# majidsina/rlmd

Hardware: NVIDIA B200
Metric: investor-steps/sec (leverage sweep) (higher is better)
Workload: dtype 2-bit codes, int32 counts, f64 log-wealth, f32 wealth

## Files before the change

rlmd_b200/csrc/common.cuh:

```cuda
#pragma once

#include <cuda_runtime.h>
#include <stdint.h>

#include <cstdarg>
#include <cstdio>

#include "../../include/rlmd_b200.h"

namespace b200 {

int set_error(int code, const char* fmt, ...);
int check_cuda(cudaError_t e, const char* what);

#define B200_CUDA(expr)                                   \
  do {                                                    \
    int _rc = ::b200::check_cuda((expr), #expr);          \
    if (_rc != 0) return _rc;                             \
  } while (0)

#define B200_REQUIRE(cond, ...)                                     \
  do {                                                              \
    if (!(cond)) return ::b200::set_error(B200_EINVAL, __VA_ARGS__); \
  } while (0)

int sm_count();

struct Philox4 {
  uint32_t x, y, z, w;
};

__host__ __device__ __forceinline__ uint32_t mulhi32(uint32_t a, uint32_t b) {
#ifdef __CUDA_ARCH__
  return __umulhi(a, b);
#else
  return (uint32_t)(((uint64_t)a * (uint64_t)b) >> 32);
#endif
}

__host__ __device__ __forceinline__ Philox4 philox4x32_10(uint32_t c0, uint32_t c1, uint32_t c2,
                                                           uint32_t c3, uint32_t k0, uint32_t k1) {
  const uint32_t M0 = 0xD2511F53u, M1 = 0xCD9E8D57u;
  const uint32_t W0 = 0x9E3779B9u, W1 = 0xBB67AE85u;
#pragma unroll
  for (int r = 0; r < 10; ++r) {
    uint32_t hi0 = mulhi32(M0, c0), lo0 = M0 * c0;
    uint32_t hi1 = mulhi32(M1, c2), lo1 = M1 * c2;
    uint32_t n0 = hi1 ^ c1 ^ k0;
    uint32_t n2 = hi0 ^ c3 ^ k1;
    c0 = n0;
    c1 = lo1;
    c2 = n2;
    c3 = lo0;
    k0 += W0;
    k1 += W1;
  }
  return Philox4{c0, c1, c2, c3};
}

// ... 150 lines not shown
```

rlmd_b200/csrc/lev_sweep.cu:

```cuda
#include <cstdlib>

#include "lev_kernels.cuh"
#include "tally.cuh"

namespace b200 {

struct LogFactorTable {
  double lm[B200_MAX_OUTCOMES][B200_MAX_GRID];
};
struct LevGrid {
  float lev[B200_MAX_GRID];
};

static int64_t out_ld(const b200_lev_desc& d) { return d.ld_out > 0 ? d.ld_out : d.n_investors; }

template <int K>
__global__ void __launch_bounds__(128)
draw_discrete_kernel(const __grid_constant__ Thresholds th, uint64_t seed, int64_t investor_offset, int32_t H,
                     int64_t N, int64_t ld, uint8_t* __restrict__ out) {
  const int nblk = (H + 3) >> 2;
  const int64_t idx = (int64_t)blockIdx.x * blockDim.x + threadIdx.x;
  if (idx >= N * nblk) return;
  const int64_t row = idx / nblk;
  const int j = (int)(idx - row * nblk);
// ... 108 lines not shown
      word |= b << (8 * i);
    }
  } else {
    for (int i = 0; i < 16; ++i) {
      const int t = w * 16 + i;
      if (t < H) word |= (uint32_t)(src[i] & 3u) << (2 * i);
    }
  }
  uint8_t* dst = packed + row * ldb + (int64_t)w * 4;
  if (w * 4 + 4 <= ldb && (((uintptr_t)dst) & 3) == 0) {
    *reinterpret_cast<uint32_t*>(dst) = word;
  } else {
    for (int b = 0; b < 4 && w * 4 + b < ldb; ++b) dst[b] = (uint8_t)(word >> (8 * b));
  }
}

template <int K>
__device__ __forceinline__ void count_word(uint32_t wd, uint32_t& s1, uint32_t& s2, uint32_t& s3) {
  s1 = __dp4a(wd & 0x01010101u, 0x01010101u, s1);
  if (K >= 3) s2 = __dp4a((wd >> 1) & 0x01010101u, 0x01010101u, s2);
  if (K >= 4) s3 = __dp4a(wd & (wd >> 1) & 0x01010101u, 0x01010101u, s3);
}

constexpr int COUNT_WARPS = 8;

template <int K>
__global__ void __launch_bounds__(COUNT_WARPS * 32)
log_discrete_stream_kernel(const uint8_t* __restrict__ outcomes, int64_t ld, int32_t H, int64_t N, int32_t G,
                           const __grid_constant__ LogFactorTable lf, double logV0, float* __restrict__ data_T,
                           double* __restrict__ log_w, int32_t* __restrict__ counts, int64_t ldT, const TallyDev tally) {
  const int lane = threadIdx.x & 31;
  const int64_t warp_global = (int64_t)blockIdx.x * COUNT_WARPS + (threadIdx.x >> 5);
  const int64_t nwarps = (int64_t)gridDim.x * COUNT_WARPS;
  for (int64_t row = warp_global; row < N; row += nwarps) {
    const uint8_t* __restrict__ p = outcomes + row * ld;
    uint32_t s1 = 0, s2 = 0, s3 = 0;
    const uintptr_t addr = (uintptr_t)p;
    int head = (int)((16 - (addr & 15)) & 15);
    if (head > H) head = H;
    const int body = (H - head) >> 4;
    const int tail0 = head + (body << 4);
    for (int t = lane; t < head; t += 32) {
      const uint32_t c = p[t];
      s1 += c & 1; if (K >= 3) s2 += (c >> 1) & 1; if (K >= 4) s3 += (c == 3);
    }
    const uint4* __restrict__ q = reinterpret_cast<const uint4*>(p + head);
    int i = lane;
    for (; i + 96 < body; i += 128) {
      const uint4 a = __ldcs(q + i), b = __ldcs(q + i + 32), c = __ldcs(q + i + 64), d = __ldcs(q + i + 96);
      count_word<K>(a.x, s1, s2, s3); count_word<K>(a.y, s1, s2, s3);
      count_word<K>(a.z, s1, s2, s3); count_word<K>(a.w, s1, s2, s3);
      count_word<K>(b.x, s1, s2, s3); count_word<K>(b.y, s1, s2, s3);
      count_word<K>(b.z, s1, s2, s3); count_word<K>(b.w, s1, s2, s3);
      count_word<K>(c.x, s1, s2, s3); count_word<K>(c.y, s1, s2, s3);
      count_word<K>(c.z, s1, s2, s3); count_word<K>(c.w, s1, s2, s3);
      count_word<K>(d.x, s1, s2, s3); count_word<K>(d.y, s1, s2, s3);
      count_word<K>(d.z, s1, s2, s3); count_word<K>(d.w, s1, s2, s3);
    }
    for (; i < body; i += 32) {
      const uint4 a = __ldcs(q + i);
      count_word<K>(a.x, s1, s2, s3); count_word<K>(a.y, s1, s2, s3);
      count_word<K>(a.z, s1, s2, s3); count_word<K>(a.w, s1, s2, s3);
    }
    for (int t = tail0 + lane; t < H; t += 32) {
      const uint32_t c = p[t];
      s1 += c & 1; if (K >= 3) s2 += (c >> 1) & 1; if (K >= 4) s3 += (c == 3);
// ... 45 lines not shown
  return make_uint4(word_mask<BITS>(valid), word_mask<BITS>(valid - PER), word_mask<BITS>(valid - 2 * PER),
                    word_mask<BITS>(valid - 3 * PER));
}

template <int K, bool TALLY, int BITS = 2>
__global__ void __launch_bounds__(COUNT_WARPS * 32, 4)
log_discrete_packed_kernel(const uint8_t* __restrict__ outcomes, int64_t ldb, int32_t H, int64_t N, int32_t G,
                           const __grid_constant__ LogFactorTable lf, double logV0, float* __restrict__ data_T,
                           double* __restrict__ log_w, int32_t* __restrict__ counts, int64_t ldT, const TallyDev tally,
                           int32_t task_rows) {
  const int lane = threadIdx.x & 31;
  const int64_t warp_global = (int64_t)blockIdx.x * COUNT_WARPS + (threadIdx.x >> 5);
  const int64_t nwarps = (int64_t)gridDim.x * COUNT_WARPS;
  constexpr int PER_BYTE = 8 / BITS;
  const int nbytes = (H + PER_BYTE - 1) / PER_BYTE;
  const int full = H / PER_BYTE;
  const int nvec = (nbytes + 15) >> 4;
  const bool vec_rows = (ldb & 15) == 0 && ldb >= (int64_t)nvec * 16;
  const int iters = (nvec + 32 * PACKED_U - 1) / (32 * PACKED_U);
  const int rem = nvec - (iters - 1) * 32 * PACKED_U;
  const int tail_slots = (rem + 31) >> 5;
  const int tail_lanes = rem - (tail_slots - 1) * 32;
  const bool in_tail = lane < tail_lanes;
  const uint4 wm = lane == tail_lanes - 1 ? last_vector_mask<BITS>(H - (128 / BITS) * (nvec - 1))
                                          : make_uint4(~0u, ~0u, ~0u, ~0u);
  auto count_byte = [&](int t, uint32_t& s1, uint32_t& s2, uint32_t& s3, const uint8_t* __restrict__ p) {
    uint32_t c = p[t];
    if (t >= full) c &= (1u << (BITS * (H % PER_BYTE))) - 1u;
    if (BITS == 1) { s1 += __popc(c); return; }
    s1 += __popc(c & 0x55u);
    if (K >= 3) s2 += __popc((c >> 1) & 0x55u);
    if (K >= 4) s3 += __popc(c & (c >> 1) & 0x55u);
  };
  for (int64_t row0 = warp_global * task_rows; row0 < N; row0 += nwarps * task_rows) {
    const int nr = (int)min((int64_t)task_rows, N - row0);
    uint32_t m1 = 0, m2 = 0, m3 = 0;
    for (int r = 0; r < nr; ++r) {
      const uint8_t* __restrict__ p = outcomes + (row0 + r) * ldb;
      uint32_t s1 = 0, s2 = 0, s3 = 0;
      if (r + 1 < nr)
        for (int b = lane * 128; b < nbytes; b += 32 * 128)
          asm volatile("prefetch.global.L2 [%0];" ::"l"(p + ldb + b));
      if (vec_rows && (((uintptr_t)p) & 15) == 0) {
        const uint4* __restrict__ q = reinterpret_cast<const uint4*>(p) + lane;
        for (int it = 0; it + 1 < iters; ++it, q += 32 * PACKED_U) {
          uint4 v[PACKED_U];
#pragma unroll
          for (int u = 0; u < PACKED_U; ++u) v[u] = __ldcs(q + u * 32);
#pragma unroll
          for (int u = 0; u < PACKED_U; ++u) {
            count_pair<K, BITS>(v[u].x, v[u].y, s1, s2, s3);
            count_pair<K, BITS>(v[u].z, v[u].w, s1, s2, s3);
          }
        }
        uint4 vl = make_uint4(0u, 0u, 0u, 0u);
        if (in_tail) vl = __ldcs(q + (tail_slots - 1) * 32);
        uint4 v[PACKED_U - 1];
#pragma unroll
        for (int u = 0; u < PACKED_U - 1; ++u)
          if (u < tail_slots - 1) v[u] = __ldcs(q + u * 32);
        vl.x &= wm.x; vl.y &= wm.y; vl.z &= wm.z; vl.w &= wm.w;
        count_pair<K, BITS>(vl.x, vl.y, s1, s2, s3);
        count_pair<K, BITS>(vl.z, vl.w, s1, s2, s3);
#pragma unroll
        for (int u = 0; u < PACKED_U - 1; ++u) {
          if (u < tail_slots - 1) {
// ... 380 lines not shown
}

static int make_log_table(const b200_lev_desc& d, const float* factors_host, LogFactorTable& lf) {
  for (int k = 0; k < B200_MAX_OUTCOMES; ++k)
    for (int g = 0; g < B200_MAX_GRID; ++g) {
      double v = 0.0;
      if (g < d.n_grid && k < d.n_outcomes) {
        const float m = factors_host[(int64_t)g * d.n_outcomes + k];
        if (m < 0.0f) return set_error(B200_EINVAL, "LOG mode needs factors >= 0 (m[%d][%d] = %g)", g, k, (double)m);
        v = log((double)m);
      }
      lf.lm[k][g] = v;
    }
  return 0;
}

static int run_log_discrete(const b200_lev_desc& d, const uint8_t* outcomes, const float* factors_host,
                            float* data_T, double* log_w, int32_t* counts, const TallyDev& tally, cudaStream_t st) {
  LogFactorTable lf;
  if (factors_host != nullptr) {
    if (int rc = make_log_table(d, factors_host, lf)) return rc;
  } else {
    memset(&lf, 0, sizeof(lf));
  }
  const double logV0 = log((double)d.value_0);
  const int64_t N = d.n_investors;
  static const int task_rows = [] { const char* e = getenv("B200_PACKED_TASK_ROWS"); int v = e ? atoi(e) : 32;
                                    return v < 1 ? 1 : v > 32 ? 32 : v; }();
  const bool packed = d.outcome_bits == 2 || d.outcome_bits == 1;
  const int64_t warps = packed ? (N + task_rows - 1) / task_rows : N;
  int64_t blocks = (warps + COUNT_WARPS - 1) / COUNT_WARPS;
  const int64_t cap = packed ? (int64_t)0x7fffffff : (int64_t)sm_count() * 8;
  if (blocks > cap) blocks = cap;
#define B200_LOG_LAUNCH(KERNEL, ...)                                                                                     \
  KERNEL<__VA_ARGS__><<<(unsigned)blocks, COUNT_WARPS * 32, 0, st>>>(outcomes, d.ld_outcomes, d.horizon, N, d.n_grid, lf, \
                                                                     logV0, data_T, log_w, counts, out_ld(d), tally B200_EXTRA)
  if (d.outcome_bits == 1) {
#define B200_EXTRA , task_rows
    if (tally.keys != nullptr) B200_LOG_LAUNCH(log_discrete_packed_kernel, 2, true, 1);
    else B200_LOG_LAUNCH(log_discrete_packed_kernel, 2, false, 1);
#undef B200_EXTRA
  } else if (d.outcome_bits == 2) {
#define B200_EXTRA , task_rows
    if (tally.keys != nullptr) {
      switch (d.n_outcomes) {
        case 2: B200_LOG_LAUNCH(log_discrete_packed_kernel, 2, true); break;
        case 3: B200_LOG_LAUNCH(log_discrete_packed_kernel, 3, true); break;
        default: B200_LOG_LAUNCH(log_discrete_packed_kernel, 4, true); break;
      }
    } else {
      switch (d.n_outcomes) {
        case 2: B200_LOG_LAUNCH(log_discrete_packed_kernel, 2, false); break;
        case 3: B200_LOG_LAUNCH(log_discrete_packed_kernel, 3, false); break;
        default: B200_LOG_LAUNCH(log_discrete_packed_kernel, 4, false); break;
      }
    }
#undef B200_EXTRA
#define B200_EXTRA
  } else {
    switch (d.n_outcomes) {
      case 2: B200_LOG_LAUNCH(log_discrete_stream_kernel, 2); break;
      case 3: B200_LOG_LAUNCH(log_discrete_stream_kernel, 3); break;
      default: B200_LOG_LAUNCH(log_discrete_stream_kernel, 4); break;
    }
  }
#undef B200_LOG_LAUNCH
#undef B200_EXTRA
  return check_cuda(cudaGetLastError(), "log_discrete_stream launch");
}

static int run_log_gbm(const b200_lev_desc& d, const float* x, const float* lev_host, float* data_T, double* log_w,
                       cudaStream_t st) {
  LevGrid lv;
  for (int g = 0; g < B200_MAX_GRID; ++g) lv.lev[g] = g < d.n_grid ? lev_host[g] : 0.f;
  const double logV0 = log((double)d.value_0);
  const int64_t N = d.n_investors;
  const bool saturate = (d.flags & B200_LEV_FLAG_FINAL_ONLY) == 0;
  const int64_t state_n = (d.flags & B200_LEV_FLAG_STATE_OUT) ? N : 0;
  if (d.source == B200_SRC_PHILOX) {
    const unsigned blocks = (unsigned)((N + 127) / 128);
    log_gbm_philox_kernel<<<blocks, 128, 0, st>>>(lv, philox_keys(d.seed), d.investor_offset, d.log_mean, d.sigma, d.horizon, N,
                                                  d.n_grid, logV0, data_T, log_w, out_ld(d), saturate, state_n);
    return check_cuda(cudaGetLastError(), "log_gbm_philox launch");
  }
  const unsigned blocks = (unsigned)((N + TILE_ROWS - 1) / TILE_ROWS);
  CUtensorMap map;
  memset(&map, 0, sizeof(map));
  if (tma_ok(x, d.ld_outcomes * 4, N)) {
    int rc = make_row_tile_map(&map, x, N, d.horizon, d.ld_outcomes, 4);
    if (rc) return rc;
    auto kern = log_gbm_stream_kernel<true>;
    B200_CUDA(cudaFuncSetAttribute(kern, cudaFuncAttributeMaxDynamicSharedMemorySize, STAGES * TILE_SMEM));
    kern<<<blocks, TILE_ROWS, STAGES * TILE_SMEM, st>>>(map, x, d.ld_outcomes, lv, d.horizon, N, d.n_grid, logV0,
                                                        data_T, log_w, out_ld(d), saturate, state_n);
  } else {
    log_gbm_stream_kernel<false><<<blocks, TILE_ROWS, TILE_SMEM, st>>>(map, x, d.ld_outcomes, lv, d.horizon, N,
                                                                       d.n_grid, logV0, data_T, log_w, out_ld(d), saturate, state_n);
  }
  return check_cuda(cudaGetLastError(), "log_gbm_stream launch");
}

// ... 337 lines not shown
```

rlmd_b200/csrc/tally.cu:

```cuda
#include <cooperative_groups.h>

#include <algorithm>
#include <cstdlib>
#include <cstring>

#include "tally.cuh"

namespace b200 {

struct BinEntry {
  unsigned long long key, count;
};
static_assert(sizeof(BinEntry) == 16, "one 16-byte vector per bin");

constexpr int MERGE_CHUNK = 2048;
constexpr int EX_FLAG_BYTES = 128;

struct LogTable {
  double lm[B200_MAX_OUTCOMES][B200_MAX_GRID];
};

struct TallyLayout {
  long long* header;
  unsigned long long* keysA; uint32_t* countsA; uint64_t capA;
  unsigned long long* ukeys; uint32_t* ucnt;
  float* wbuf; int64_t ldw;
  int64_t list_cap;
  BinEntry* concat; uint32_t* slot_of;
  unsigned long long* keysB; unsigned long long* countsB; uint32_t* posB; uint64_t capB;
  int32_t* blockcnt; int64_t nblk;
  int64_t bytes;
};

static uint64_t pow2_at_least(uint64_t v) {
  uint64_t p = 1;
  while (p < v) p <<= 1;
  return p;
}

static int plan_ok(const b200_tally_plan* p) {
  B200_REQUIRE(p != nullptr, "tally: plan is NULL");
  B200_REQUIRE(p->rows_cap >= 1 && p->rows_cap < ((int64_t)1 << 32), "tally: rows_cap must be in 1..2^32-1");
  B200_REQUIRE(p->bins_cap >= 1 && p->bins_cap < ((int64_t)1 << 31), "tally: bins_cap must be in 1..2^31-1");
  B200_REQUIRE(p->grid_cap >= 1 && p->grid_cap <= B200_MAX_GRID, "tally: grid_cap must be in 1..%d", B200_MAX_GRID);
  B200_REQUIRE(p->world >= 1 && p->world <= B200_MAX_PEERS, "tally: world must be in 1..%d", B200_MAX_PEERS);
  return 0;
}

static TallyLayout layout(const b200_tally_plan& p, void* base) {
  TallyLayout L;
  memset(&L, 0, sizeof(L));
  char* b = (char*)base;
  int64_t off = 0;
  auto take = [&](int64_t bytes) { char* r = b ? b + off : nullptr; off += (bytes + 255) & ~(int64_t)255; return r; };
  L.header = (long long*)take(TH_WORDS * 8);
  L.capA = pow2_at_least((uint64_t)std::max<int64_t>(2048, 2 * std::min(p.rows_cap, p.bins_cap)));
  L.list_cap = (int64_t)(L.capA / 2);
  L.keysA = (unsigned long long*)take((int64_t)L.capA * 8);
  L.countsA = (uint32_t*)take((int64_t)L.capA * 4);
  L.ukeys = (unsigned long long*)take(p.bins_cap * 8);
  L.ucnt = (uint32_t*)take(p.bins_cap * 4);
  L.ldw = (p.bins_cap + 3) & ~(int64_t)3;
  L.wbuf = (float*)take((int64_t)p.grid_cap * L.ldw * 4);
  if (p.world > 1) {
    const int64_t cat = (int64_t)p.world * L.list_cap;
    L.concat = (BinEntry*)take(cat * 16);
    L.slot_of = (uint32_t*)take(cat * 4);
    L.capB = pow2_at_least((uint64_t)std::max<int64_t>(1024, 2 * std::min(cat, p.bins_cap)));
    L.keysB = (unsigned long long*)take((int64_t)L.capB * 8);
    L.countsB = (unsigned long long*)take((int64_t)L.capB * 8);
    L.posB = (uint32_t*)take((int64_t)L.capB * 4);
    L.nblk = (cat + MERGE_CHUNK - 1) / MERGE_CHUNK;
    L.blockcnt = (int32_t*)take(L.nblk * 4);
  }
  L.bytes = off;
  return L;
}

static int64_t exchange_list_bytes(int64_t list_cap) { return 16 + list_cap * 16; }

int tally_device_view(const b200_tally_plan* plan, void* workspace, int32_t horizon, TallyDev* out) {
  if (int rc = plan_ok(plan)) return rc;
  B200_REQUIRE(workspace != nullptr, "tally: workspace is NULL");
  B200_REQUIRE(horizon <= TALLY_MAX_HORIZON, "tally: horizon must be < 2^%d (use b200_lev_sweep + b200_rowstats)",
               TALLY_COUNT_BITS);
  const TallyLayout L = layout(*plan, workspace);
  out->keys = L.keysA;
  out->counts = L.countsA;
  out->header = L.header;
  out->mask = L.capA - 1;
  return 0;
}

__global__ void __launch_bounds__(256)
tally_clear_kernel(unsigned long long* keys, uint32_t* counts32, unsigned long long* counts64, uint32_t* pos,
                   uint64_t cap) {
  for (uint64_t i = (uint64_t)blockIdx.x * blockDim.x + threadIdx.x; i < cap; i += (uint64_t)gridDim.x * blockDim.x) {
    keys[i] = TALLY_EMPTY;
    if (counts32) counts32[i] = 0;
    if (counts64) counts64[i] = 0;
    if (pos) pos[i] = 0xffffffffu;
  }
}

struct PeerView {
  BinEntry* list[B200_MAX_PEERS];
  long long* list_count[B200_MAX_PEERS];
  uint32_t* flags[B200_MAX_PEERS];
  int32_t world, rank;
  uint32_t epoch;
};

__device__ __forceinline__ void box_add(uint32_t (&b)[4], unsigned long long key) {
  int n1, n2, n3;
  tally_unkey(key, n1, n2, n3);
  b[0] = max(b[0], (uint32_t)(TALLY_MAX_HORIZON - n1)); b[1] = max(b[1], (uint32_t)n1);
  b[2] = max(b[2], (uint32_t)(TALLY_MAX_HORIZON - n2)); b[3] = max(b[3], (uint32_t)n2);
}
__device__ __forceinline__ void box_flush(const uint32_t (&b)[4], long long* dst, uint32_t* s ) {
  if (threadIdx.x < 4) s[threadIdx.x] = 0;
  __syncthreads();
#pragma unroll
  for (int q = 0; q < 4; ++q) {
    const uint32_t m = __reduce_max_sync(0xffffffffu, b[q]);
    if ((threadIdx.x & 31) == 0 && m != 0u) atomicMax(s + q, m);
  }
  __syncthreads();
  if (threadIdx.x < 4 && s[threadIdx.x] != 0u)
    atomicMax(reinterpret_cast<unsigned long long*>(dst) + threadIdx.x, (unsigned long long)s[threadIdx.x]);
}

constexpr int COMPACT_PER = 8;
constexpr int COMPACT_CHUNK = 256 * COMPACT_PER;

template <bool MULTI>
__global__ void __launch_bounds__(256)
tally_compact_kernel(TallyDev t, unsigned long long* __restrict__ ukeys, uint32_t* __restrict__ ucnt,
                     int64_t out_cap, const __grid_constant__ PeerView P) {
  __shared__ BinEntry stage[COMPACT_CHUNK];
  __shared__ int n_s;
  __shared__ long long base_s;
  __shared__ uint32_t box_s[4];
  uint32_t box[4] = {0, 0, 0, 0};
  const uint64_t cap = t.mask + 1;
  const uint64_t base = (uint64_t)blockIdx.x * COMPACT_CHUNK;
  if (threadIdx.x == 0) n_s = 0;
  __syncthreads();
  unsigned long long key[COMPACT_PER];
  uint32_t cnt[COMPACT_PER];
#pragma unroll
  for (int u = 0; u < COMPACT_PER; ++u) {
    const uint64_t i = base + (uint64_t)u * 256 + threadIdx.x;
    key[u] = i < cap ? __ldcg(t.keys + i) : TALLY_EMPTY;
    cnt[u] = i < cap ? __ldcg(t.counts + i) : 0u;
  }
#pragma unroll
  for (int u = 0; u < COMPACT_PER; ++u) {
    if (key[u] == TALLY_EMPTY) continue;
    const uint64_t i = base + (uint64_t)u * 256 + threadIdx.x;
    t.keys[i] = TALLY_EMPTY;
    t.counts[i] = 0;
    if (!MULTI) box_add(box, key[u]);
    const int p = atomicAdd(&n_s, 1);
    stage[p].key = key[u];
    stage[p].count = cnt[u];
  }
  __syncthreads();
  const int n = n_s;
  if (!MULTI && n > 0) box_flush(box, t.header + TH_BOX_ACC, box_s);
  if (n > 0) {
    if (threadIdx.x == 0)
      base_s = (long long)atomicAdd(reinterpret_cast<unsigned long long*>(t.header + TH_LISTPOS), (unsigned long long)n);
    __syncthreads();
    BinEntry* list = MULTI ? P.list[P.rank] : nullptr;
    for (int j = threadIdx.x; j < n; j += 256) {
      const long long p = base_s + j;
      if (p < out_cap) {
        if (MULTI) list[p] = stage[j];
        else { ukeys[p] = stage[j].key; ucnt[p] = (uint32_t)stage[j].count; }
      } else {
        t.header[TH_OVERFLOW] = 1;
      }
    }
  }
  __shared__ int last_s;
  __threadfence();
  __syncthreads();
  if (threadIdx.x == 0) {
    const unsigned long long tk = atomicAdd(reinterpret_cast<unsigned long long*>(t.header + TH_TICKET), 1ull);
    last_s = tk == (unsigned long long)gridDim.x - 1;
  }
  __syncthreads();
  if (!last_s) return;
  __threadfence();
  if (threadIdx.x == 0) {
    const long long total = *reinterpret_cast<volatile long long*>(t.header + TH_LISTPOS);
    const long long m = total < out_cap ? total : out_cap;
    t.header[TH_LISTPOS] = 0;
    t.header[TH_TICKET] = 0;
    if (MULTI) *P.list_count[P.rank] = m;
    else {
      t.header[TH_NBINS] = m;
      t.header[TH_RADIX] = 0;
      for (int q = 0; q < 4; ++q) {
        t.header[TH_BOX + q] = *reinterpret_cast<volatile long long*>(t.header + TH_BOX_ACC + q);
        t.header[TH_BOX_ACC + q] = 0;
      }
    }
  }
  if (MULTI) {
    __syncthreads();
    if (threadIdx.x < P.world && threadIdx.x != P.rank) {
      __threadfence_system();
      uint32_t* f = P.flags[threadIdx.x] + P.rank;
      asm volatile("st.release.sys.global.u32 [%0], %1;" ::"l"(f), "r"(P.epoch) : "memory");
    }
  }
}

__device__ __forceinline__ void ld_sys_entry(const BinEntry* p, unsigned long long& k, unsigned long long& c) {
  asm volatile("ld.relaxed.sys.global.v2.u64 {%0, %1}, [%2];" : "=l"(k), "=l"(c) : "l"(p));
}

__global__ void __launch_bounds__(256)
tally_merge_kernel(const __grid_constant__ PeerView P, long long* __restrict__ header, BinEntry* __restrict__ concat,
                   uint32_t* __restrict__ slot_of, unsigned long long* __restrict__ keysB,
                   unsigned long long* __restrict__ countsB, uint32_t* __restrict__ posB, uint64_t capB,
                   int64_t concat_cap) {
  __shared__ long long off_s[B200_MAX_PEERS + 1];
  __shared__ int ok_s;
  if (threadIdx.x == 0) ok_s = 1;
  __syncthreads();
  if (threadIdx.x < P.world && threadIdx.x != P.rank) {
    const uint32_t* f = P.flags[P.rank] + threadIdx.x;
    unsigned long long t0, t1;
    asm volatile("mov.u64 %0, %%globaltimer;" : "=l"(t0));
    for (;;) {
      uint32_t v;
      asm volatile("ld.acquire.sys.global.u32 %0, [%1];" : "=r"(v) : "l"(f) : "memory");
      if ((int32_t)(v - P.epoch) >= 0) break;
      __nanosleep(100);
      asm volatile("mov.u64 %0, %%globaltimer;" : "=l"(t1));
      if (t1 - t0 > 30000000000ull) { ok_s = 0; break; }
    }
  }
  __syncthreads();
  if (!ok_s) {
    if (threadIdx.x == 0) { header[TH_TIMEOUT] = 1; header[TH_CONCAT] = 0; }
// ... 224 lines not shown
  for (int q = 0; q < N; ++q) v[q] = warp_sum(v[q]);
  __syncthreads();
  if (lane == 0)
#pragma unroll
    for (int q = 0; q < N; ++q) scratch[q * 32 + wid] = v[q];
  __syncthreads();
  if (wid == 0) {
#pragma unroll
    for (int q = 0; q < N; ++q) {
      const double x = lane < (int)(blockDim.x >> 5) ? scratch[q * 32 + lane] : 0.0;
      v[q] = warp_sum(x);
    }
  }
}

template <int NK>
__global__ void __launch_bounds__(SEL_THREADS)
tally_select_kernel(long long* __restrict__ header, const unsigned long long* __restrict__ ukeys,
                    const uint32_t* __restrict__ ucnt, float* __restrict__ wbuf, int64_t ldw, int32_t H,
                    const __grid_constant__ LogTable lf, double logV0, int64_t n_total, int64_t top,
                    double* __restrict__ stats, int32_t SEL_CACHE ,
                    int32_t force_radix) {
  namespace cg = cooperative_groups;
  cg::cluster_group cluster = cg::this_cluster();
  const int C = (int)cluster.num_blocks(), r = (int)cluster.block_rank();
  __shared__ SelShared sh;
  extern __shared__ __align__(16) uint8_t dyn[];
  float* cw = reinterpret_cast<float*>(dyn);
  uint32_t* cc = reinterpret_cast<uint32_t*>(dyn) + SEL_CACHE;
  uint16_t* cb = reinterpret_cast<uint16_t*>(cc + SEL_CACHE);
  SelShared* L = cluster.map_shared_rank(&sh, 0);

  const int g = blockIdx.x / C;
  const long long B = header[TH_NBINS];
  const long long n = n_total, K = top;
  const double qnan = __longlong_as_double(0x7ff8000000000000LL);
  double* s = stats + (int64_t)g * 12;
  if (header[TH_TIMEOUT] != 0 || header[TH_OVERFLOW] != 0) {
    if (r == 0 && threadIdx.x < 12) s[threadIdx.x] = qnan;
    return;
  }
  const int tid = threadIdx.x, lane = threadIdx.x & 31;
#ifdef B200_TALLY_DEBUG
  int stamp_i = 0;
#define STAMP() do { if (r == 0 && tid == 0 && (g == 0 || g == (int)(gridDim.x / C) - 1)) { header[TH_DEBUG + (g == 0 ? 0 : 24) + stamp_i++] = clock64(); } } while (0)
#else
#define STAMP() do {} while (0)
#endif
  STAMP();
  const long long per = (((B + C - 1) / C) + 3) & ~3LL;
  const long long lo = min(B, (long long)r * per), hi = min(B, lo + per);
  const int m = (int)(hi - lo);
  float* __restrict__ w = wbuf + (int64_t)g * ldw + lo;
  const uint32_t* __restrict__ cnt = ucnt + lo;
  constexpr int REGS = 0;
  double lm[NK];
#pragma unroll
  for (int k = 0; k < NK; ++k) lm[k] = lf.lm[k][g];
  auto lw_of = [&](unsigned long long key) {
    int n1, n2, n3;
    tally_unkey(key, n1, n2, n3);
    int nk[4];
    nk[1] = n1; nk[2] = NK >= 3 ? n2 : 0; nk[3] = NK >= 4 ? n3 : 0;
    nk[0] = H - nk[1] - nk[2] - nk[3];
    double lw = logV0;
#pragma unroll
// ... 480 lines not shown
  }();
  static int k = [] {
    const char* e = getenv("B200_SELECT_CACHE");
    int x = e ? atoi(e) : 16384;
    return x < 0 ? 0 : x > 20480 ? 20480 : x;
  }();
  cluster = c;
  cache = k;
}

template <int K>
static int launch_select_k(int n_grid, long long* header, const unsigned long long* ukeys, const uint32_t* ucnt,
                           float* wbuf, int64_t ldw, int32_t H, const LogTable& lf, double logV0, int64_t n_total,
                           int64_t top, double* stats, bool beside_sweep, bool force_radix, cudaStream_t st) {
  static bool attr_set[64] = {false};
  int dev = 0;
  B200_CUDA(cudaGetDevice(&dev));
  int C = 1, cache = 0;
  select_shape(C, cache);
  static const bool forced = getenv("B200_SELECT_CLUSTER") != nullptr;
  if (beside_sweep && !forced) C = 2;
  const size_t dyn = (size_t)cache * 10;
  if (dev < 64 && !attr_set[dev]) {
    B200_CUDA(cudaFuncSetAttribute(tally_select_kernel<K>, cudaFuncAttributeMaxDynamicSharedMemorySize, (int)dyn));
    if (C > 8) B200_CUDA(cudaFuncSetAttribute(tally_select_kernel<K>, cudaFuncAttributeNonPortableClusterSizeAllowed, 1));
    attr_set[dev] = true;
  }
  cudaLaunchConfig_t cfg;
  memset(&cfg, 0, sizeof(cfg));
  cfg.gridDim = dim3((unsigned)(n_grid * C));
  cfg.blockDim = dim3(SEL_THREADS);
  cfg.dynamicSmemBytes = dyn;
  cfg.stream = st;
  cudaLaunchAttribute at[1];
  at[0].id = cudaLaunchAttributeClusterDimension;
  at[0].val.clusterDim.x = (unsigned)C;
  at[0].val.clusterDim.y = 1;
  at[0].val.clusterDim.z = 1;
  cfg.attrs = at;
  cfg.numAttrs = 1;
  return check_cuda(cudaLaunchKernelEx(&cfg, tally_select_kernel<K>, header, ukeys, ucnt, wbuf, ldw, H, lf, logV0,
                                       n_total, top, stats, (int32_t)cache, (int32_t)force_radix),
                    "tally_select launch");
}

static int grid_for(int64_t work, int threads, int per_sm) {
  const int64_t want = (work + threads - 1) / threads;
  const int64_t cap = (int64_t)sm_count() * per_sm;
  return (int)std::max<int64_t>(1, std::min(want, cap));
}

}

using namespace b200;

extern "C" int64_t b200_tally_workspace_bytes(const b200_tally_plan* plan) {
  if (plan_ok(plan)) return -1;
  return layout(*plan, nullptr).bytes;
}

extern "C" int64_t b200_tally_exchange_bytes(const b200_tally_plan* plan) {
  if (plan_ok(plan)) return -1;
  if (plan->world == 1) return 0;
  const TallyLayout L = layout(*plan, nullptr);
  return EX_FLAG_BYTES + 2 * ((exchange_list_bytes(L.list_cap) + 255) & ~(int64_t)255);
}

extern "C" int b200_tally_reset(const b200_tally_plan* plan, void* workspace, void* stream) {
  if (int rc = plan_ok(plan)) return rc;
  B200_REQUIRE(workspace != nullptr, "tally_reset: workspace is NULL");
  cudaStream_t st = (cudaStream_t)stream;
  const TallyLayout L = layout(*plan, workspace);
  B200_CUDA(cudaMemsetAsync(L.header, 0, TH_WORDS * 8, st));
  tally_clear_kernel<<<grid_for((int64_t)L.capA, 256, 8), 256, 0, st>>>(L.keysA, L.countsA, nullptr, nullptr, L.capA);
  if (plan->world > 1)
    tally_clear_kernel<<<grid_for((int64_t)L.capB, 256, 8), 256, 0, st>>>(L.keysB, nullptr, L.countsB, L.posB, L.capB);
  return check_cuda(cudaGetLastError(), "tally_reset launch");
}

extern "C" int b200_tally_finalize(const b200_tally_plan* plan, void* workspace, const b200_tally_peers* peers,
                                   int32_t phase, void* stream) {
  if (int rc = plan_ok(plan)) return rc;
  B200_REQUIRE(workspace != nullptr, "tally_finalize: workspace is NULL");
  B200_REQUIRE(phase >= -1 && phase <= 1, "tally_finalize: phase must be -1, 0 or 1");
  cudaStream_t st = (cudaStream_t)stream;
  const TallyLayout L = layout(*plan, workspace);
  TallyDev t{L.keysA, L.countsA, L.header, L.capA - 1};
  PeerView P;
  memset(&P, 0, sizeof(P));
  const int cgrid = (int)((L.capA + COMPACT_CHUNK - 1) / COMPACT_CHUNK);
  if (plan->world == 1) {
    if (phase == 1) return 0;
    tally_compact_kernel<false><<<cgrid, 256, 0, st>>>(t, L.ukeys, L.ucnt, std::min(plan->bins_cap, L.list_cap), P);
    return check_cuda(cudaGetLastError(), "tally_compact launch");
  }
  B200_REQUIRE(peers != nullptr, "tally_finalize: peers is NULL with world > 1");
  B200_REQUIRE(peers->world == plan->world && peers->rank >= 0 && peers->rank < peers->world,
               "tally_finalize: peers->world / rank do not fit the plan");
  B200_REQUIRE(peers->epoch >= 1, "tally_finalize: epoch starts at 1");
  const int64_t lbytes = (exchange_list_bytes(L.list_cap) + 255) & ~(int64_t)255;
  P.world = peers->world; P.rank = peers->rank; P.epoch = peers->epoch;
  for (int r = 0; r < peers->world; ++r) {
    B200_REQUIRE(peers->exchange[r] != nullptr, "tally_finalize: exchange buffer of rank %d is NULL", r);
    char* ex = (char*)peers->exchange[r];
    char* lst = ex + EX_FLAG_BYTES + (peers->epoch & 1) * lbytes;
    P.flags[r] = (uint32_t*)ex;
    P.list_count[r] = (long long*)lst;
    P.list[r] = (BinEntry*)(lst + 16);
  }
  if (phase != 1) {
    tally_compact_kernel<true><<<cgrid, 256, 0, st>>>(t, nullptr, nullptr, L.list_cap, P);
    B200_CUDA(cudaGetLastError());
  }
  if (phase == 0) return 0;
  const int64_t cat = (int64_t)plan->world * L.list_cap;
  tally_merge_kernel<<<sm_count() * 2, 256, 0, st>>>(P, L.header, L.concat, L.slot_of, L.keysB, L.countsB, L.posB,
                                                     L.capB, cat);
  B200_CUDA(cudaGetLastError());
  const unsigned mgrid = (unsigned)std::min<int64_t>(L.nblk, (int64_t)sm_count() * 2);
  tally_mark_kernel<<<mgrid, 256, 0, st>>>(L.header, L.slot_of, L.posB, L.blockcnt);
  B200_CUDA(cudaGetLastError());
  tally_unique_kernel<<<mgrid, 256, 0, st>>>(L.header, L.concat, L.slot_of, L.keysB, L.countsB, L.posB,
                                                        L.blockcnt, L.ukeys, L.ucnt, plan->bins_cap);
  return check_cuda(cudaGetLastError(), "tally_unique launch");
}

extern "C" int b200_tally_stats(const b200_tally_plan* plan, void* workspace, const b200_lev_desc* desc,
                                const float* factors_host, int64_t n_total, int64_t top, double* stats, void* stream) {
  if (int rc = plan_ok(plan)) return rc;
  B200_REQUIRE(workspace != nullptr && desc != nullptr && factors_host != nullptr && stats != nullptr,
               "tally_stats: NULL argument");
  B200_REQUIRE(desc->n_grid >= 1 && desc->n_grid <= plan->grid_cap, "tally_stats: n_grid must be in 1..grid_cap");
  B200_REQUIRE(desc->n_outcomes >= 2 && desc->n_outcomes <= B200_MAX_OUTCOMES, "tally_stats: n_outcomes out of range");
  B200_REQUIRE(desc->horizon >= 1 && desc->horizon <= TALLY_MAX_HORIZON, "tally_stats: horizon out of range");
  B200_REQUIRE(n_total >= 2 && n_total < ((int64_t)1 << 32), "tally_stats: need 2 <= n_total < 2^32");
  B200_REQUIRE(top >= 1 && top < n_total, "tally_stats: need 1 <= top < n_total (top=%lld)", (long long)top);
  cudaStream_t st = (cudaStream_t)stream;
  const TallyLayout L = layout(*plan, workspace);
  LogTable lf;
  for (int k = 0; k < B200_MAX_OUTCOMES; ++k)
    for (int g = 0; g < B200_MAX_GRID; ++g) {
      double v = 0.0;
      if (g < desc->n_grid && k < desc->n_outcomes) {
        const float m = factors_host[(int64_t)g * desc->n_outcomes + k];
// ... 15 lines not shown
```

rlmd_b200/csrc/tally.cuh:

```cuda
#pragma once
#include "common.cuh"

namespace b200 {

constexpr unsigned long long TALLY_EMPTY = ~0ull;
constexpr int TALLY_COUNT_BITS = 21;
constexpr int64_t TALLY_MAX_HORIZON = (1 << TALLY_COUNT_BITS) - 1;

enum {
  TH_NBINS = 0,
  TH_OVERFLOW = 1,
  TH_BAD = 2,
  TH_TIMEOUT = 3,
  TH_MISMATCH = 4,
  TH_RADIX = 5,
  TH_TICKET = 9,
  TH_LISTPOS = 10,
  TH_CONCAT = 11,
  TH_DEBUG = 16,
  TH_BOX_ACC = 64,
  TH_BOX = 68,
  TH_WORDS = 72
};

struct TallyDev {
  unsigned long long* keys;
  uint32_t* counts;
  long long* header;
  uint64_t mask;
};

__host__ __device__ __forceinline__ uint64_t tally_mix(uint64_t x) {
  x ^= x >> 33; x *= 0xff51afd7ed558ccdull;
  x ^= x >> 33; x *= 0xc4ceb9fe1a85ec53ull;
  x ^= x >> 33;
  return x;
}

__host__ __device__ __forceinline__ uint64_t tally_key(int n1, int n2, int n3) {
  return (uint64_t)(uint32_t)n1 | ((uint64_t)(uint32_t)n2 << TALLY_COUNT_BITS) |
         ((uint64_t)(uint32_t)n3 << (2 * TALLY_COUNT_BITS));
}
__host__ __device__ __forceinline__ void tally_unkey(uint64_t key, int& n1, int& n2, int& n3) {
  n1 = (int)(key & TALLY_MAX_HORIZON);
  n2 = (int)((key >> TALLY_COUNT_BITS) & TALLY_MAX_HORIZON);
  n3 = (int)((key >> (2 * TALLY_COUNT_BITS)) & TALLY_MAX_HORIZON);
}

constexpr int TALLY_MAX_PROBE = 256;
__device__ __forceinline__ void tally_insert(const TallyDev& t, uint64_t key, uint32_t add) {
  uint64_t slot = tally_mix(key) & t.mask;
  for (int probe = 0; probe < TALLY_MAX_PROBE; ++probe) {
    unsigned long long cur = __ldcg(t.keys + slot);
    if (cur == TALLY_EMPTY) {
      cur = atomicCAS(t.keys + slot, TALLY_EMPTY, (unsigned long long)key);
      if (cur == TALLY_EMPTY) cur = key;
    }
    if (cur == key) { atomicAdd(t.counts + slot, add); return; }
    slot = (slot + 1) & t.mask;
  }
  t.header[TH_OVERFLOW] = 1;
}

int tally_device_view(const ::b200_tally_plan* plan, void* workspace, int32_t horizon, TallyDev* out);

}
```

Baseline: 21970 billion.

## Record claimed tally slots and gather them instead of scanning table; add PDL launches

New measurement: 22070 billion (median of 6 runs). No clear change (+0.5%).

```diff
diff --git a/rlmd_b200/csrc/common.cuh b/rlmd_b200/csrc/common.cuh
--- a/rlmd_b200/csrc/common.cuh
+++ b/rlmd_b200/csrc/common.cuh
@@ -25,6 +25,23 @@
   } while (0)
 
 int sm_count();
+
+__device__ __forceinline__ void griddep_wait() { asm volatile("griddepcontrol.wait;" ::: "memory"); }
+
+template <typename... P, typename... A>
+cudaError_t launch_pdl(void (*kernel)(P...), dim3 grid, dim3 block, size_t smem, cudaStream_t st, A&&... args) {
+  cudaLaunchConfig_t cfg = {};
+  cfg.gridDim = grid;
+  cfg.blockDim = block;
+  cfg.dynamicSmemBytes = smem;
+  cfg.stream = st;
+  cudaLaunchAttribute at[1];
+  at[0].id = cudaLaunchAttributeProgrammaticStreamSerialization;
+  at[0].val.programmaticStreamSerializationAllowed = 1;
+  cfg.attrs = at;
+  cfg.numAttrs = 1;
+  return cudaLaunchKernelEx(&cfg, kernel, static_cast<A&&>(args)...);
+}
 
 struct Philox4 {
   uint32_t x, y, z, w;
diff --git a/rlmd_b200/csrc/lev_sweep.cu b/rlmd_b200/csrc/lev_sweep.cu
--- a/rlmd_b200/csrc/lev_sweep.cu
+++ b/rlmd_b200/csrc/lev_sweep.cu
@@ -164,6 +164,7 @@
   const int lane = threadIdx.x & 31;
   const int64_t warp_global = (int64_t)blockIdx.x * COUNT_WARPS + (threadIdx.x >> 5);
   const int64_t nwarps = (int64_t)gridDim.x * COUNT_WARPS;
+  griddep_wait();
   for (int64_t row = warp_global; row < N; row += nwarps) {
     const uint8_t* __restrict__ p = outcomes + row * ld;
     uint32_t s1 = 0, s2 = 0, s3 = 0;
@@ -275,6 +276,7 @@
     if (K >= 3) s2 += __popc((c >> 1) & 0x55u);
     if (K >= 4) s3 += __popc(c & (c >> 1) & 0x55u);
   };
+  griddep_wait();
   for (int64_t row0 = warp_global * task_rows; row0 < N; row0 += nwarps * task_rows) {
     const int nr = (int)min((int64_t)task_rows, N - row0);
     uint32_t m1 = 0, m2 = 0, m3 = 0;
@@ -721,9 +723,10 @@
   int64_t blocks = (warps + COUNT_WARPS - 1) / COUNT_WARPS;
   const int64_t cap = packed ? (int64_t)0x7fffffff : (int64_t)sm_count() * 8;
   if (blocks > cap) blocks = cap;
-#define B200_LOG_LAUNCH(KERNEL, ...)                                                                                     \
-  KERNEL<__VA_ARGS__><<<(unsigned)blocks, COUNT_WARPS * 32, 0, st>>>(outcomes, d.ld_outcomes, d.horizon, N, d.n_grid, lf, \
-                                                                     logV0, data_T, log_w, counts, out_ld(d), tally B200_EXTRA)
+  cudaError_t le = cudaSuccess;
+#define B200_LOG_LAUNCH(KERNEL, ...)                                                                               \
+  le = launch_pdl(KERNEL<__VA_ARGS__>, dim3((unsigned)blocks), dim3(COUNT_WARPS * 32), 0, st, outcomes,            \
+                  d.ld_outcomes, d.horizon, N, d.n_grid, lf, logV0, data_T, log_w, counts, out_ld(d), tally B200_EXTRA)
   if (d.outcome_bits == 1) {
 #define B200_EXTRA , task_rows
     if (tally.keys != nullptr) B200_LOG_LAUNCH(log_discrete_packed_kernel, 2, true, 1);
@@ -755,7 +758,7 @@
   }
 #undef B200_LOG_LAUNCH
 #undef B200_EXTRA
-  return check_cuda(cudaGetLastError(), "log_discrete_stream launch");
+  return check_cuda(le != cudaSuccess ? le : cudaGetLastError(), "log_discrete_stream launch");
 }
 
 static int run_log_gbm(const b200_lev_desc& d, const float* x, const float* lev_host, float* data_T, double* log_w,
diff --git a/rlmd_b200/csrc/tally.cu b/rlmd_b200/csrc/tally.cu
--- a/rlmd_b200/csrc/tally.cu
+++ b/rlmd_b200/csrc/tally.cu
@@ -26,6 +26,7 @@
   unsigned long long* ukeys; uint32_t* ucnt;
   float* wbuf; int64_t ldw;
   int64_t list_cap;
+  uint32_t* claimed; unsigned long long* cursors; uint32_t sub_cap;
   BinEntry* concat; uint32_t* slot_of;
   unsigned long long* keysB; unsigned long long* countsB; uint32_t* posB; uint64_t capB;
   int32_t* blockcnt; int64_t nblk;
@@ -62,6 +63,11 @@
   L.ucnt = (uint32_t*)take(p.bins_cap * 4);
   L.ldw = (p.bins_cap + 3) & ~(int64_t)3;
   L.wbuf = (float*)take((int64_t)p.grid_cap * L.ldw * 4);
+  if (p.world == 1) {
+    L.sub_cap = (uint32_t)(L.capA / TALLY_SUBLISTS);
+    L.claimed = (uint32_t*)take((int64_t)TALLY_SUBLISTS * L.sub_cap * 4);
+    L.cursors = (unsigned long long*)take((int64_t)TALLY_SUBLISTS * TALLY_CURSOR_STRIDE * 8);
+  }
   if (p.world > 1) {
     const int64_t cat = (int64_t)p.world * L.list_cap;
     L.concat = (BinEntry*)take(cat * 16);
@@ -89,6 +95,9 @@
   out->counts = L.countsA;
   out->header = L.header;
   out->mask = L.capA - 1;
+  out->claimed = L.claimed;
+  out->cursors = L.cursors;
+  out->sub_cap = L.sub_cap;
   return 0;
 }
 
@@ -133,15 +142,11 @@
 constexpr int COMPACT_PER = 8;
 constexpr int COMPACT_CHUNK = 256 * COMPACT_PER;
 
-template <bool MULTI>
 __global__ void __launch_bounds__(256)
-tally_compact_kernel(TallyDev t, unsigned long long* __restrict__ ukeys, uint32_t* __restrict__ ucnt,
-                     int64_t out_cap, const __grid_constant__ PeerView P) {
+tally_compact_kernel(TallyDev t, int64_t out_cap, const __grid_constant__ PeerView P) {
   __shared__ BinEntry stage[COMPACT_CHUNK];
   __shared__ int n_s;
   __shared__ long long base_s;
-  __shared__ uint32_t box_s[4];
-  uint32_t box[4] = {0, 0, 0, 0};
   const uint64_t cap = t.mask + 1;
   const uint64_t base = (uint64_t)blockIdx.x * COMPACT_CHUNK;
   if (threadIdx.x == 0) n_s = 0;
@@ -160,24 +165,21 @@
     const uint64_t i = base + (uint64_t)u * 256 + threadIdx.x;
     t.keys[i] = TALLY_EMPTY;
     t.counts[i] = 0;
-    if (!MULTI) box_add(box, key[u]);
     const int p = atomicAdd(&n_s, 1);
     stage[p].key = key[u];
     stage[p].count = cnt[u];
   }
   __syncthreads();
   const int n = n_s;
-  if (!MULTI && n > 0) box_flush(box, t.header + TH_BOX_ACC, box_s);
   if (n > 0) {
     if (threadIdx.x == 0)
       base_s = (long long)atomicAdd(reinterpret_cast<unsigned long long*>(t.header + TH_LISTPOS), (unsigned long long)n);
     __syncthreads();
-    BinEntry* list = MULTI ? P.list[P.rank] : nullptr;
+    BinEntry* list = P.list[P.rank];
     for (int j = threadIdx.x; j < n; j += 256) {
       const long long p = base_s + j;
       if (p < out_cap) {
-        if (MULTI) list[p] = stage[j];
-        else { ukeys[p] = stage[j].key; ucnt[p] = (uint32_t)stage[j].count; }
+        list[p] = stage[j];
       } else {
         t.header[TH_OVERFLOW] = 1;
       }
@@ -198,22 +200,80 @@
     const long long m = total < out_cap ? total : out_cap;
     t.header[TH_LISTPOS] = 0;
     t.header[TH_TICKET] = 0;
-    if (MULTI) *P.list_count[P.rank] = m;
-    else {
-      t.header[TH_NBINS] = m;
-      t.header[TH_RADIX] = 0;
-      for (int q = 0; q < 4; ++q) {
-        t.header[TH_BOX + q] = *reinterpret_cast<volatile long long*>(t.header + TH_BOX_ACC + q);
-        t.header[TH_BOX_ACC + q] = 0;
-      }
-    }
-  }
-  if (MULTI) {
-    __syncthreads();
-    if (threadIdx.x < P.world && threadIdx.x != P.rank) {
-      __threadfence_system();
-      uint32_t* f = P.flags[threadIdx.x] + P.rank;
-      asm volatile("st.release.sys.global.u32 [%0], %1;" ::"l"(f), "r"(P.epoch) : "memory");
+    *P.list_count[P.rank] = m;
+  }
+  __syncthreads();
+  if (threadIdx.x < P.world && threadIdx.x != P.rank) {
+    __threadfence_system();
+    uint32_t* f = P.flags[threadIdx.x] + P.rank;
+    asm volatile("st.release.sys.global.u32 [%0], %1;" ::"l"(f), "r"(P.epoch) : "memory");
+  }
+}
+
+constexpr int GATHER_THREADS = 256;
+
+__global__ void __launch_bounds__(GATHER_THREADS)
+tally_gather_kernel(TallyDev t, unsigned long long* __restrict__ ukeys, uint32_t* __restrict__ ucnt, int64_t out_cap) {
+  __shared__ long long off_s[TALLY_SUBLISTS + 1];
+  __shared__ uint32_t box_s[4];
+  __shared__ int last_s;
+  uint32_t box[4] = {0, 0, 0, 0};
+  griddep_wait();
+  static_assert(TALLY_SUBLISTS == 64, "one warp scans two sub-lists per lane");
+  if (threadIdx.x < 32) {
+    const int l = threadIdx.x;
+    const unsigned long long a = __ldcg(t.cursors + (2 * l) * TALLY_CURSOR_STRIDE);
+    const unsigned long long b = __ldcg(t.cursors + (2 * l + 1) * TALLY_CURSOR_STRIDE);
+    const long long ca = (long long)a, cb = (long long)b;
+    long long incl = ca + cb;
+#pragma unroll
+    for (int o = 1; o < 32; o <<= 1) {
+      const long long up = __shfl_up_sync(0xffffffffu, incl, o);
+      if (l >= o) incl += up;
+    }
+    off_s[2 * l] = incl - ca - cb;
+    off_s[2 * l + 1] = incl - cb;
+    if (l == 31) off_s[TALLY_SUBLISTS] = incl;
+  }
+  __syncthreads();
+  const long long total = off_s[TALLY_SUBLISTS];
+  for (long long i = (long long)blockIdx.x * GATHER_THREADS + threadIdx.x; i < total;
+       i += (long long)gridDim.x * GATHER_THREADS) {
+    int s = 0;
+#pragma unroll
+    for (int step = TALLY_SUBLISTS / 2; step > 0; step >>= 1)
+      if (off_s[s + step] <= i) s += step;
+    const uint32_t slot = t.claimed[(uint64_t)s * t.sub_cap + (uint64_t)(i - off_s[s])];
+    const unsigned long long key = __ldcg(t.keys + slot);
+    const uint32_t cnt = __ldcg(t.counts + slot);
+    t.keys[slot] = TALLY_EMPTY;
+    t.counts[slot] = 0;
+    if (i < out_cap) {
+      box_add(box, key);
+      ukeys[i] = key;
+      ucnt[i] = cnt;
+    } else {
+      t.header[TH_OVERFLOW] = 1;
+    }
+  }
+  box_flush(box, t.header + TH_BOX_ACC, box_s);
+  __threadfence();
+  __syncthreads();
+  if (threadIdx.x == 0) {
+    const unsigned long long tk = atomicAdd(reinterpret_cast<unsigned long long*>(t.header + TH_TICKET), 1ull);
+    last_s = tk == (unsigned long long)gridDim.x - 1;
+  }
+  __syncthreads();
+  if (!last_s) return;
+  __threadfence();
+  if (threadIdx.x < TALLY_SUBLISTS) t.cursors[threadIdx.x * TALLY_CURSOR_STRIDE] = 0;
+  if (threadIdx.x == 0) {
+    t.header[TH_NBINS] = total < out_cap ? total : out_cap;
+    t.header[TH_RADIX] = 0;
+    t.header[TH_TICKET] = 0;
+    for (int q = 0; q < 4; ++q) {
+      t.header[TH_BOX + q] = *reinterpret_cast<volatile long long*>(t.header + TH_BOX_ACC + q);
+      t.header[TH_BOX_ACC + q] = 0;
     }
   }
 }
@@ -504,6 +564,7 @@
   SelShared* L = cluster.map_shared_rank(&sh, 0);
 
   const int g = blockIdx.x / C;
+  griddep_wait();
   const long long B = header[TH_NBINS];
   const long long n = n_total, K = top;
   const double qnan = __longlong_as_double(0x7ff8000000000000LL);
@@ -1050,13 +1111,15 @@
   cfg.blockDim = dim3(SEL_THREADS);
   cfg.dynamicSmemBytes = dyn;
   cfg.stream = st;
-  cudaLaunchAttribute at[1];
+  cudaLaunchAttribute at[2];
   at[0].id = cudaLaunchAttributeClusterDimension;
   at[0].val.clusterDim.x = (unsigned)C;
   at[0].val.clusterDim.y = 1;
   at[0].val.clusterDim.z = 1;
+  at[1].id = cudaLaunchAttributeProgrammaticStreamSerialization;
+  at[1].val.programmaticStreamSerializationAllowed = 1;
   cfg.attrs = at;
-  cfg.numAttrs = 1;
+  cfg.numAttrs = 2;
   return check_cuda(cudaLaunchKernelEx(&cfg, tally_select_kernel<K>, header, ukeys, ucnt, wbuf, ldw, H, lf, logV0,
                                        n_total, top, stats, (int32_t)cache, (int32_t)force_radix),
                     "tally_select launch");
@@ -1090,6 +1153,7 @@
   cudaStream_t st = (cudaStream_t)stream;
   const TallyLayout L = layout(*plan, workspace);
   B200_CUDA(cudaMemsetAsync(L.header, 0, TH_WORDS * 8, st));
+  if (L.cursors) B200_CUDA(cudaMemsetAsync(L.cursors, 0, TALLY_SUBLISTS * TALLY_CURSOR_STRIDE * 8, st));
   tally_clear_kernel<<<grid_for((int64_t)L.capA, 256, 8), 256, 0, st>>>(L.keysA, L.countsA, nullptr, nullptr, L.capA);
   if (plan->world > 1)
     tally_clear_kernel<<<grid_for((int64_t)L.capB, 256, 8), 256, 0, st>>>(L.keysB, nullptr, L.countsB, L.posB, L.capB);
@@ -1103,14 +1167,16 @@
   B200_REQUIRE(phase >= -1 && phase <= 1, "tally_finalize: phase must be -1, 0 or 1");
   cudaStream_t st = (cudaStream_t)stream;
   const TallyLayout L = layout(*plan, workspace);
-  TallyDev t{L.keysA, L.countsA, L.header, L.capA - 1};
+  TallyDev t{L.keysA, L.countsA, L.header, L.capA - 1, L.claimed, L.cursors, L.sub_cap};
   PeerView P;
   memset(&P, 0, sizeof(P));
-  const int cgrid = (int)((L.capA + COMPACT_CHUNK - 1) / COMPACT_CHUNK);
   if (plan->world == 1) {
     if (phase == 1) return 0;
-    tally_compact_kernel<false><<<cgrid, 256, 0, st>>>(t, L.ukeys, L.ucnt, std::min(plan->bins_cap, L.list_cap), P);
-    return check_cuda(cudaGetLastError(), "tally_compact launch");
+    const int64_t out_cap = std::min(plan->bins_cap, L.list_cap);
+    const unsigned ggrid = (unsigned)grid_for(out_cap, GATHER_THREADS, 2);
+    return check_cuda(launch_pdl(tally_gather_kernel, dim3(ggrid), dim3(GATHER_THREADS), 0, st, t, L.ukeys, L.ucnt,
+                                 out_cap),
+                      "tally_gather launch");
   }
   B200_REQUIRE(peers != nullptr, "tally_finalize: peers is NULL with world > 1");
   B200_REQUIRE(peers->world == plan->world && peers->rank >= 0 && peers->rank < peers->world,
@@ -1127,7 +1193,8 @@
     P.list[r] = (BinEntry*)(lst + 16);
   }
   if (phase != 1) {
-    tally_compact_kernel<true><<<cgrid, 256, 0, st>>>(t, nullptr, nullptr, L.list_cap, P);
+    const int cgrid = (int)((L.capA + COMPACT_CHUNK - 1) / COMPACT_CHUNK);
+    tally_compact_kernel<<<cgrid, 256, 0, st>>>(t, L.list_cap, P);
     B200_CUDA(cudaGetLastError());
   }
   if (phase == 0) return 0;
diff --git a/rlmd_b200/csrc/tally.cuh b/rlmd_b200/csrc/tally.cuh
--- a/rlmd_b200/csrc/tally.cuh
+++ b/rlmd_b200/csrc/tally.cuh
@@ -23,11 +23,17 @@
   TH_WORDS = 72
 };
 
+constexpr int TALLY_SUBLISTS = 64;
+constexpr int TALLY_CURSOR_STRIDE = 16;
+
 struct TallyDev {
   unsigned long long* keys;
   uint32_t* counts;
   long long* header;
   uint64_t mask;
+  uint32_t* claimed;
+  unsigned long long* cursors;
+  uint32_t sub_cap;
 };
 
 __host__ __device__ __forceinline__ uint64_t tally_mix(uint64_t x) {
@@ -54,7 +60,14 @@
     unsigned long long cur = __ldcg(t.keys + slot);
     if (cur == TALLY_EMPTY) {
       cur = atomicCAS(t.keys + slot, TALLY_EMPTY, (unsigned long long)key);
-      if (cur == TALLY_EMPTY) cur = key;
+      if (cur == TALLY_EMPTY) {
+        cur = key;
+        if (t.claimed != nullptr) {
+          const uint32_t s = (uint32_t)slot & (TALLY_SUBLISTS - 1);
+          const unsigned long long p = atomicAdd(t.cursors + s * TALLY_CURSOR_STRIDE, 1ull);
+          t.claimed[(uint64_t)s * t.sub_cap + p] = (uint32_t)slot;
+        }
+      }
     }
     if (cur == key) { atomicAdd(t.counts + slot, add); return; }
     slot = (slot + 1) & t.mask;
```
